# PlakarLabs/plakar

Measured on AMD Instinct MI355X. Metric: GiB/s chunked (device-resident, cut-points out) at 1/2/4/8 MI355X, higher is better.
Workload: dtype u8; 1 GPU; C1: 1x 1 GiB uniform random buffer per GPU (BASELINE configs[1]); bytes_per_gpu=1073741824, global_bytes=1073741824, buffers_per_gpu=1, chunk_params=FASTCDC min 65536 / normal 1048576 / max 4194304, gear=placeholder (v0.0.8 table unavailable; see DESIGN.md), parallelism=independent buffers, 1 rank per GPU x 1, no collective, streams=2

## Files before the change

plakar_amd/csrc/cdc_kernels.hip:

```cpp
#include <hip/hip_ext.h>
#include <hip/hip_runtime.h>

#include <algorithm>
#include <mutex>
#include <type_traits>
#include <vector>

#include "cdc_hostmem.h"
#include "cdc_internal.h"

namespace cdc {

#ifndef CDC_SPIN_SLEEP
#define CDC_SPIN_SLEEP 1
#endif
constexpr int kSpinSleep = CDC_SPIN_SLEEP;

static constexpr uint64_t kNoHit = ~0ull;
static constexpr uint32_t kRawLaneBytes = 512;
static constexpr uint32_t kWarm = 64;

template <int NT, int COPIES = 32>
__device__ __forceinline__ void fill_gear_lds(uint64_t *tab, const uint64_t *gear, uint32_t sh = 0)
{
    static_assert(NT % 64 == 0, "block size");
    constexpr uint32_t kSlots = 256u * COPIES;
    constexpr int kPer = int((kSlots + NT - 1) / NT);
    uint64_t v[kPer];
#pragma unroll
    for (int i = 0; i < kPer; ++i) {
        const uint32_t x = threadIdx.x + uint32_t(i) * NT;
        v[i] = x < kSlots ? gear[x / COPIES] : 0;
    }
#pragma unroll
    for (int i = 0; i < kPer; ++i) {
        const uint32_t x = threadIdx.x + uint32_t(i) * NT;
        if (x < kSlots) tab[x] = v[i] << sh;
    }
}
constexpr uint32_t kWCopies = 8;
constexpr uint32_t kWEntShift = kWCopies == 32 ? 8 : kWCopies == 16 ? 7 : 6;
static_assert(kWCopies == 8 || kWCopies == 16 || kWCopies == 32, "walker table copies");

__device__ __forceinline__ uint64_t lds_gear(const char *tab, uint32_t addr)
{
    return *reinterpret_cast<const uint64_t *>(tab + addr);
}

typedef __attribute__((address_space(3))) const char lds_char;
typedef __attribute__((address_space(1))) const uint64_t g_u64;
typedef __attribute__((address_space(1))) const uint32_t g_u32;
typedef __attribute__((address_space(1))) const uint8_t g_u8;

__device__ __forceinline__ uint64_t lds_gear(const lds_char *tab, uint32_t addr)
{
    return *reinterpret_cast<__attribute__((address_space(3))) const uint64_t *>(tab + addr);
}

template <typename T>
__device__ __forceinline__ T *as_space(uint64_t addr)
{
    return reinterpret_cast<T *>(uintptr_t(addr));
}

__device__ __forceinline__ const lds_char *as_lds(const char *p)
{
    return as_space<const lds_char>(uint32_t(reinterpret_cast<uintptr_t>(p)));
}

__device__ __forceinline__ uint4 gload16(uint64_t a)
{
    const g_u64 *q = as_space<const g_u64>(a);
    const uint64_t x = q[0], y = q[1];
    return make_uint4(uint32_t(x), uint32_t(x >> 32), uint32_t(y), uint32_t(y >> 32));
}

__device__ __forceinline__ uint32_t gear_addr(uint32_t laneoff, uint32_t word, int k)
{
    return __builtin_amdgcn_perm(laneoff, word, 0x0C0C0004u | (uint32_t(k & 3) << 8));
}

template <uint32_t ESH = kWEntShift>
__device__ __forceinline__ uint32_t wgear_addr(uint32_t wlaneoff, uint32_t word, int k)
{
    if constexpr (ESH == 8) return gear_addr(wlaneoff, word, k);
    return (__builtin_amdgcn_ubfe(word, uint32_t(k & 3) * 8u, 8u) << ESH) | wlaneoff;
}

__device__ __forceinline__ uint32_t key_of(uint64_t fp, uint32_t mlo, uint32_t mhi)
{
    return __builtin_amdgcn_bitop3_b32(uint32_t(fp >> 32), mhi, uint32_t(fp) & mlo, 0xEA);
}

__device__ __forceinline__ uint32_t word_of(const uint4 &d, int i)
{
    return i == 0 ? d.x : i == 1 ? d.y : i == 2 ? d.z : d.w;
}

__device__ __forceinline__ uint32_t umin3(uint32_t a, uint32_t b, uint32_t c)
{
    uint32_t r;
    asm("v_min3_u32 %0, %1, %2, %3" : "=v"(r) : "v"(a), "v"(b), "v"(c));
    return r;
}

template <uint32_t ESH = kWEntShift, typename TP>
__device__ __forceinline__ uint32_t roll16_test(const uint4 &d, uint64_t &fp, TP tab,
                                                uint32_t laneoff, uint32_t mlo, uint32_t mhi)
{
    uint32_t acc = 0xFFFFFFFFu;
#pragma unroll
    for (int k = 0; k < 16; ++k) {
        fp = (fp << 1) + lds_gear(tab, wgear_addr<ESH>(laneoff, word_of(d, k >> 2), k));
        acc = min(acc, key_of(fp, mlo, mhi));
    }
    return acc;
}

template <uint32_t ESH = kWEntShift, typename TP>
__device__ __forceinline__ void roll16(const uint4 &d, uint64_t &fp, TP tab,
                                       uint32_t laneoff)
{
#pragma unroll
    for (int k = 0; k < 16; ++k)
        fp = (fp << 1) + lds_gear(tab, wgear_addr<ESH>(laneoff, word_of(d, k >> 2), k));
}

template <uint32_t ESH = kWEntShift, typename TP>
__device__ __forceinline__ uint64_t group_first_hit(const uint4 &d, uint64_t &fp, uint64_t a,
                                                    uint64_t ts, uint64_t te, uint64_t fz,
                                                    TP tab, uint32_t laneoff,
                                                    uint32_t mlo, uint32_t mhi)
// ... 121 lines not shown
    const uint64_t base = (uint64_t(uint32_t(__builtin_amdgcn_readfirstlane(uint32_t(base_in >> 32)))) << 32) |
                          uint32_t(__builtin_amdgcn_readfirstlane(uint32_t(base_in)));
    const uint32_t dst = __builtin_amdgcn_readfirstlane(dst_in);
    uint32_t keep;
    asm volatile("s_nop 4\n\ts_mov_b32 %[keep], m0\n\ts_mov_b32 m0, %[dst]\n\ts_nop 0\n\t"
                 DMA_PIECE_IMM(1, 0) DMA_PIECE_IMM(2, 1024) DMA_PIECE_IMM(3, 2048) DMA_PIECE_IMM(4, 3072)
                 "s_mov_b32 m0, %[keep]\n\ts_nop 1"
                 : [keep] "=&s"(keep)
                 : "v"(offi[0]), "v"(offi[1]), "v"(offi[2]), "v"(offi[3]), [base] "s"(base), [dst] "s"(dst)
                 : "memory");
}

__device__ __forceinline__ uint32_t wave_ticket(uint32_t *p)
{
    const uint32_t old = __hip_atomic_fetch_add(p, (threadIdx.x & 63u) == 0u ? 1u : 0u, __ATOMIC_RELAXED,
                                                __HIP_MEMORY_SCOPE_AGENT);
    return __builtin_amdgcn_readfirstlane(old);
}

__device__ __forceinline__ uint32_t scan_wave_max(uint32_t v)
{
#pragma unroll
    for (int o = 32; o; o >>= 1) v = max(v, uint32_t(__shfl_xor(int(v), o)));
    return __builtin_amdgcn_readfirstlane(v);
}

__device__ __forceinline__ uint32_t rec_cnt(uint64_t rec) { return uint32_t(rec & ((1u << kRecCntBits) - 1)); }
__device__ __forceinline__ uint32_t rec_ent(uint64_t rec, uint32_t e)
{
    return uint32_t(rec >> (kRecCntBits + kRecEntBits * e)) & ((1u << kRecEntBits) - 1);
}

__device__ __forceinline__ void record_hit(uint64_t &rec, int32_t r)
{
    const uint32_t c = rec_cnt(rec);
    if (c < kRunCap) rec |= uint64_t(uint32_t(r)) << (kRecCntBits + kRecEntBits * c);
    if (c < (1u << kRecCntBits) - 1) ++rec;
}

constexpr uint64_t kMaskLSpill = 16;

__device__ bool maskl_needed(const Batch &B, const DevParams &P, const Workspace &W, const BufDesc &D, uint64_t t,
                             uint32_t lane)
{
    const uint64_t sl = B.scan_lane, tb = 64ull * sl;
    const uint64_t start = t * tb, end = min(D.len, start + tb);
    const uint64_t ra = start / sl, rb = (end - 1) / sl;
    const uint64_t gap = P.normal_size - P.min_size - (P.win - 1);
    const uint32_t kc = uint32_t(gap / sl > 2 ? gap / sl - 1 : 1);
    const uint64_t r_lo = ra > kc + kMaskLSpill ? ra - kc - kMaskLSpill : 0;
    const uint64_t *runs = W.runs + 64ull * D.task_base;
    uint32_t cur = 0;
    for (uint64_t r4 = r_lo; r4 <= rb; r4 += 256) {
        uint64_t rec[4];
#pragma unroll
        for (int j = 0; j < 4; ++j) {
            const uint64_t q = r4 + 64u * j + lane;
            rec[j] = q <= rb ? runs[q] : 1ull;
        }
#pragma unroll
        for (int j = 0; j < 4; ++j) {
            const uint64_t r0 = r4 + 64u * j;
            if (r0 > rb) break;
            const uint64_t E = __ballot(rec_cnt(rec[j]) == 0);
            const uint32_t n = uint32_t(min(rb + 1 - r0, uint64_t(64)));
            const uint64_t Z = ~E & (n == 64 ? ~0ull : (1ull << n) - 1);
            const uint64_t below = Z & ((1ull << lane) - 1);
            const uint32_t prev = below ? lane - 1u - (63u - uint32_t(__builtin_clzll(below))) : cur + lane;
            const uint64_t r = r0 + lane;
            bool need = false;
            if (lane < n) {
                if ((E >> lane) & 1ull)
                    need = r >= ra && prev + 1 >= kc;
                else
                    need = prev >= kc && r + kMaskLSpill >= ra;
            }
            if (__ballot(need)) return true;
            cur = Z ? n - 1u - (63u - uint32_t(__builtin_clzll(Z))) : cur + n;
        }
    }
    return false;
}

template <bool kMaskL, bool kFused>
__device__ __forceinline__ void scan_task(const Batch &B, const DevParams &P, const Workspace &W, char *s_lds,
                                          const char *tab, uint32_t task, uint32_t lane, uint32_t wave,
                                          uint32_t laneoff);

template <bool kMaskL, bool kFused = false>
__device__ __forceinline__ void scan_body(const Batch &B, const DevParams &P, const Workspace &W)
{
    static_assert(!(kMaskL && kFused), "k_scan_f builds both indexes, from the MaskS records' side");
    __shared__ __attribute__((aligned(16)))
    char s_lds[kGearLdsBytes + kS2Waves * (kStageBytes + kQBytes) + (kFused ? kFlushTabBytes : 0u)];
    const uint32_t lane = threadIdx.x & 63u;
    const uint32_t wave = __builtin_amdgcn_readfirstlane(threadIdx.x >> 6);
    const uint32_t laneoff = (lane & 31u) << 3;
    const uint32_t task = blockIdx.x * kS2Waves + wave;
    bool act = true;
    if constexpr (kMaskL) {
        act = false;
        if (task < B.total_tasks) {
            uint32_t bb = 0;
            while (bb + 1 < B.nbufs && task >= B.b[bb + 1].task_base) ++bb;
            const BufDesc &Db = B.b[bb];
            const uint64_t t = task - Db.task_base;
            if (t * 64ull * B.scan_lane < Db.len) act = maskl_needed(B, P, W, Db, t, lane);
            if (lane == 0) W.validL[task] = act ? 1u : 0u;
        }
        if (!__syncthreads_or(act ? 1 : 0)) return;
        if (threadIdx.x == 0 && B.maskl_hint)
            __hip_atomic_store(B.maskl_hint, 1u, __ATOMIC_RELAXED, __HIP_MEMORY_SCOPE_SYSTEM);
    }
    if constexpr (!kMaskL) {
        const uint32_t gt = blockIdx.x * blockDim.x + threadIdx.x, nth = gridDim.x * blockDim.x;
        for (uint32_t i = gt; i < B.total_segs; i += nth) {
            W.xg[i] = 0ull;
            W.sg[i] = 0ull;
        }
        if (gt < kMaxBufsPerLaunch + 4)
            W.flags[gt] = gt == kLimitWord ? uint32_t(B.spin_ticks ? B.spin_ticks : kSpinLimit) : 0u;
        if (gt < 2) W.tick[gt] = 0u;
        if (gt < B.nbufs) B.b[gt].res->status = kRowPending;
        if (threadIdx.x == 0) dbg_ts(B, kTsScan + 4 * blockIdx.x);
    }
    uint32_t clk = 0;
    if (!kMaskL && (B.debug & kDbgClk) && blockIdx.x == 0 && threadIdx.x == 0) {
        clk = kTsClk + 4u * uint32_t(atomicAdd(reinterpret_cast<unsigned long long *>(&g_ts[kTsClkN]), 1ull) % kClkRecs);
        g_ts[clk] = __builtin_amdgcn_s_memrealtime();
        g_ts[clk + 1] = __builtin_amdgcn_s_memtime();
    }
    fill_gear_lds<kS2Waves * 64>(reinterpret_cast<uint64_t *>(s_lds), W.gear,
                                 kFused ? P.fm_sh : kMaskL ? P.fl_sh : P.fs_sh);
    if constexpr (kFused) {
        static_assert(kS2Waves * 64 >= 256, "one entry per thread");
        if (threadIdx.x < 256)
            reinterpret_cast<uint64_t *>(s_lds + kGearLdsBytes + kS2Waves * (kStageBytes + kQBytes))[threadIdx.x] =
                W.gear[threadIdx.x] << P.fs_sh;
    }
    __syncthreads();
    if (!kMaskL && threadIdx.x == 0) {
        dbg_ts(B, kTsScan + 4 * blockIdx.x + 1);
        if (blockIdx.x < 4096)
            dbg_ts(B, kTsHw + blockIdx.x,
                   uint64_t(__builtin_amdgcn_s_getreg(20 | (0 << 6) | (15 << 11))) << 32 |
                       uint32_t(__builtin_amdgcn_s_getreg(4 | (0 << 6) | (31 << 11))));
    }
    const char *tab = s_lds;
    if (!act) return;
    const bool persist = !kMaskL && B.persist != 0;
    auto next_task = [&]() { return wave_ticket(W.tick + 2); };
    for (uint32_t cur = persist ? next_task() : task;;) {
        if (cur >= B.total_tasks) break;
        scan_task<kMaskL, kFused>(B, P, W, s_lds, tab, cur, lane, wave, laneoff);
        if (!persist) break;
        cur = next_task();
    }
    if (clk && threadIdx.x == 0) {
        g_ts[clk + 2] = __builtin_amdgcn_s_memrealtime();
        g_ts[clk + 3] = __builtin_amdgcn_s_memtime();
    }
}

template <bool kMaskL, bool kFused>
__device__ __forceinline__ void scan_task(const Batch &B, const DevParams &P, const Workspace &W, char *s_lds,
                                          const char *tab, uint32_t task, uint32_t lane, uint32_t wave,
                                          uint32_t laneoff)
{
    uint32_t b = 0;
    while (b + 1 < B.nbufs && task >= B.b[b + 1].task_base) ++b;
    const BufDesc &D = B.b[b];

    const uint64_t sl = B.scan_lane;
    const uint64_t ub = reinterpret_cast<uint64_t>(D.data);
    const uint64_t lo_ok = ub & ~15ull, hi_ok = (ub + D.len + 15) & ~15ull;
    const uint64_t seg0 = uint64_t(task - D.task_base) * 64u;
    if (seg0 * sl >= D.len) return;
    const int64_t s = int64_t((seg0 + lane) * sl);
    constexpr uint32_t kLead = 128u;
    const uint32_t T = uint32_t((sl + kLead + (ub & 15u) + kStage - 1u) / kStage);
    const uint64_t wb = ((ub + seg0 * sl) & ~15ull) - kLead;
    const uint64_t base = wb > lo_ok ? wb : lo_ok;
    const uint64_t limw = hi_ok - 16u - base;
    const uint32_t lim = limw > 0x7FFFFFFFull ? 0x7FFFFFFFu : uint32_t(limw);
    const uint32_t ring = uint32_t(reinterpret_cast<uintptr_t>(s_lds)) + kGearLdsBytes + wave * kStageBytes;
    static_assert(kStage == 64 && kL == 4, "pair staging: 64-B stages, one slot");
    const uint32_t half = lane >> 5;
    const uint32_t row = lane & 31u, swz = (row >> 1) & 7u;
    uint32_t offi[4];
    uint32_t om = 0;
#pragma unroll
    for (uint32_t j = 0; j < 4; ++j) {
        const uint32_t r = 8u * j + lane / 8u;
        const uint32_t k = (lane % 8u) ^ ((r >> 1) & 7u);
        const uint32_t o = uint32_t((((ub + (seg0 + r) * sl) & ~15ull) - kLead + 16u * k) - base);
        om = max(om, o);
        offi[j] = o - 1024u * j;
    }
    const uint64_t om0 = scan_wave_max(om);
    const uint64_t half_step = 32ull * sl;
    auto issue = [&](auto PC, uint32_t u, auto FC) {
        constexpr uint32_t Q = decltype(PC)::value;
        constexpr bool kFast = decltype(FC)::value;
        const uint64_t adv = uint64_t(kStage) * (u - Q) + (Q ? half_step : 0ull);
#ifdef CDC_DIAG_NO_DMA
        return;
#endif
        if (kFast || om0 + adv <= uint64_t(lim)) {
#ifdef CDC_DIAG_L2
            dma_stage_imm(lo_ok + ((base + adv - lo_ok) & 0x7FFF0ull), ring, offi);
#else
            dma_stage_imm(base + adv, ring, offi);
#endif
        } else {
            uint32_t eff[4];
#pragma unroll
            for (uint32_t j = 0; j < 4; ++j) eff[j] = min(offi[j] + 1024u * j + uint32_t(adv), lim);
            dma_stage(base, ring, eff);
        }
    };
    const char *rowp = s_lds + kGearLdsBytes + wave * kStageBytes + row * 128u;
    auto load_row = [&](uint4 (&first)[4], uint4 (&second)[4]) {
#ifdef CDC_DIAG_NO_ROW
        asm volatile("" : "+v"(first[0].x), "+v"(second[0].x));
        return;
#endif
#pragma unroll
        for (uint32_t g = 0; g < 4; ++g) first[g] = *reinterpret_cast<const uint4 *>(rowp + 16u * (g ^ swz));
#pragma unroll
        for (uint32_t g = 0; g < 4; ++g) second[g] = *reinterpret_cast<const uint4 *>(rowp + 16u * ((g + 4) ^ swz));
    };
    const uint32_t TT = T + 1;
    const int32_t lag = int32_t(kStage * half);
    const uint32_t vhi = to_vgpr(kFused ? P.fm_mi : kMaskL ? P.fl_hi : P.fs_hi);
    const uint32_t xlo = kMaskL ? P.fl_lo : P.fs_lo, xhi = kMaskL ? P.fl_hi : P.fs_hi;
    const int64_t rel0 = int64_t(((ub + uint64_t(s)) & ~15ull) - kLead) - int64_t(ub);
    using C0 = std::integral_constant<uint32_t, 0>;
    using C1 = std::integral_constant<uint32_t, 1>;
    using Gen = std::integral_constant<bool, false>;
    using Steady = std::integral_constant<bool, true>;

    uint4 A[4] = {}, Bv[4] = {};
#ifdef CDC_DIAG_WAITS
    uint64_t wsum = 0;
    uint32_t nrc = 0;
    const uint64_t tk0 = __builtin_amdgcn_s_memtime();
    const uint64_t rt0 = __builtin_amdgcn_s_memrealtime();
#endif
    static_assert(kLead >= 2 * kStage, "stage 0 must be pure warm-up for both halves");
    issue(C0{}, 0, Gen{});
    wait_vmcnt<0>();
    if (half == 0) load_row(A, Bv);
    asm volatile("s_waitcnt lgkmcnt(0)" ::: "memory");
    if (1 < TT) issue(C1{}, 1, Gen{});
    if (1 < TT) {
        wait_vmcnt<0>();
        if (half == 1) load_row(Bv, A);
        asm volatile("s_waitcnt lgkmcnt(0)" ::: "memory");
        if (2 < TT) issue(C0{}, 2, Gen{});
    }
    uint64_t gv[2][16];
#pragma unroll
    for (int k = 0; k < 16; ++k) gv[0][k] = lds_gear(tab, gear_addr(laneoff, word_of(Bv[0], k >> 2), k));
    uint64_t fp = 0;
    uint64_t rec = 0;
    uint64_t recL = 0;
    const int32_t rr0 = int32_t(rel0 - s) - lag;
    uint64_t *const qf = reinterpret_cast<uint64_t *>(s_lds + kGearLdsBytes + kS2Waves * kStageBytes + wave * kQBytes);
    uint32_t *const qm = reinterpret_cast<uint32_t *>(qf + kQCap);
    static_assert(kQCap == 64, "one flush pass: item j in lane j");
    uint32_t qn = 0;
    const char *const ftab = s_lds + kGearLdsBytes + kS2Waves * (kStageBytes + kQBytes);
    auto rgear = [&](const uint4 &d, int k) -> uint64_t {
        if constexpr (kFused)
            return lds_gear(ftab, __builtin_amdgcn_ubfe(word_of(d, k >> 2), uint32_t(k & 3) * 8u, 8u) << 3);
        else
            return lds_gear(tab, gear_addr(laneoff, word_of(d, k >> 2), k));
    };
    auto flush = [&]() {
        {
            const bool v = lane < qn;
            const uint32_t meta = qm[v ? lane : 0u];
            const uint32_t owner = meta >> 24;
            const int32_t r0 = int32_t(meta & 0xFFFFFFu) - 256;
            const int64_t so = int64_t((seg0 + owner) * sl);
            const int32_t ln = so < int64_t(D.len) ? int32_t(min(int64_t(sl), int64_t(D.len) - so)) : 0;
            const uint64_t a = ub + uint64_t(so + r0);
            auto clamp16 = [&](uint64_t x) { return min(max(x, lo_ok), hi_ok - 16u); };
            const uint4 d0 = gload16(clamp16(a)), d1 = gload16(clamp16(a + 16u));
            uint64_t f = 0;
            if constexpr (kFused) {
                uint4 dw[4];
#pragma unroll
                for (int h = 0; h < 4; ++h) dw[h] = gload16(clamp16(a - 64u + 16u * uint32_t(h)));
#pragma unroll
                for (int k = 0; k < 64; ++k) f = (f << 1) + rgear(dw[k >> 4], k & 15);
            } else {
                f = qf[v ? lane : 0u];
            }
            uint32_t miss = 0, missL = 0;
#pragma unroll
            for (int k = 0; k < 32; ++k) {
                f = (f << 1) + rgear(k < 16 ? d0 : d1, k & 15);
                miss |= min(key_of(f, xlo, xhi), 1u) << k;
                if constexpr (kFused) missL |= min(key_of(f, P.fm_llo, P.fm_lhi), 1u) << k;
            }
            const int32_t lo = r0 < 0 ? -r0 : 0, hi = ln - r0;
            uint32_t vm = lo >= 32 ? 0u : (0xFFFFFFFFu << lo);
            vm &= hi >= 32 ? 0xFFFFFFFFu : (hi <= 0 ? 0u : (1u << hi) - 1u);
            const uint32_t hm = v ? ~miss & vm : 0u;
            const uint32_t hmL = kFused && v ? ~missL & vm : 0u;
            uint64_t todo = __ballot(hm != 0 || hmL != 0);
            while (todo) {
                const int i = int(__builtin_ctzll(todo));
                todo &= todo - 1;
                const uint32_t o = uint32_t(__builtin_amdgcn_readlane(int(owner), i));
                const int32_t ri = __builtin_amdgcn_readlane(r0, i);
                uint32_t m = uint32_t(__builtin_amdgcn_readlane(int(hm), i));
                uint32_t mL = kFused ? uint32_t(__builtin_amdgcn_readlane(int(hmL), i)) : 0u;
                if (lane == o) {
                    for (; m; m &= m - 1) record_hit(rec, ri + int32_t(__builtin_ctz(m)));
                    if constexpr (kFused)
                        for (; mL; mL &= mL - 1) record_hit(recL, ri + int32_t(__builtin_ctz(mL)));
                }
            }
        }
        qn = 0;
    };
    uint64_t f0 = 0;
    uint32_t acc = 0xFFFFFFFFu;
    auto stage = [&](auto PC, auto SC, uint32_t t, uint4 (&cur_d)[4], uint4 (&nxt_d)[4]) {
        constexpr uint32_t Q = decltype(PC)::value;
        constexpr bool kSteady = decltype(SC)::value;
#pragma unroll
        for (uint32_t gi = 0; gi < kGroups; ++gi) {
            if (gi + 1 == kGroups && (kSteady || t + 1 < TT)) {
#ifdef CDC_DIAG_WAITS
                const uint64_t w0 = __builtin_amdgcn_s_memtime();
                wait_vmcnt<0>();
                wsum += __builtin_amdgcn_s_memtime() - w0;
#else
                wait_vmcnt<0>();
#endif
                if (half != Q) load_row(nxt_d, cur_d);
                asm volatile("" ::: "memory");
            }
            const uint4 nx = gi + 1 < kGroups ? cur_d[gi + 1] : nxt_d[0];
            uint64_t (&cg)[16] = gv[gi & 1];
            uint64_t (&ng)[16] = gv[(gi + 1) & 1];
            if ((gi & 1) == 0) {
                f0 = fp;
                acc = 0xFFFFFFFFu;
            }
#pragma unroll
            for (int q = 0; q < 4; ++q) {
#pragma unroll
                for (int k = 4 * q; k < 4 * q + 4; k += 2) {
                    const uint32_t a0 = gear_addr(laneoff, word_of(nx, k >> 2), k);
                    fp = (fp << 1) + cg[k];
                    ng[k] = lds_gear(tab, a0);
                    const uint32_t k0 = uint32_t(fp >> 32) & vhi;
                    const uint32_t a1 = gear_addr(laneoff, word_of(nx, (k + 1) >> 2), k + 1);
                    fp = (fp << 1) + cg[k + 1];
                    ng[k + 1] = lds_gear(tab, a1);
                    acc = umin3(acc, k0, uint32_t(fp >> 32) & vhi);
                    __builtin_amdgcn_sched_barrier(0);
                }
                __builtin_amdgcn_sched_barrier(0);
                if (q == 1 && gi + 1 == kGroups && (kSteady || t + 2 < TT)) {
                    asm volatile("s_waitcnt lgkmcnt(8)" ::: "memory");
                    issue(PC, t + 2, SC);
                    __builtin_amdgcn_sched_barrier(0);
                }
            }
            if (gi & 1) {
#ifndef CDC_DIAG_NO_RECHECK
                const uint64_t fm = __ballot(acc == 0);
#ifdef CDC_DIAG_WAITS
                nrc += fm ? 1u : 0u;
#endif
                if (fm) [[unlikely]] {
                    const uint32_t nq = uint32_t(__popcll(fm));
                    if (qn + nq > kQCap) flush();
                    if (acc == 0) {
                        const uint32_t idx =
                            qn + __builtin_amdgcn_mbcnt_hi(uint32_t(fm >> 32), __builtin_amdgcn_mbcnt_lo(uint32_t(fm), 0u));
                        const int32_t r0 = rr0 + int32_t(kStage * t + 16u * (gi - 1));
                        if constexpr (!kFused) qf[idx] = f0;
                        qm[idx] = uint32_t(r0 + 256) | (lane << 24);
                    }
                    qn += nq;
                }
#else
                rec += acc == 0 ? 1u : 0u;
#endif
            }
        }
    };
    if (1 < TT) stage(C1{}, Gen{}, 1, Bv, A);
    const int64_t room = int64_t(lim) - int64_t(om0) - int64_t(half_step);
    const int64_t tf = room >= 128 ? room / 64 - 1 : 0;
    const uint32_t t_steady = uint32_t(max<int64_t>(2, min<int64_t>(int64_t(TT) - 3, tf)));
    uint32_t t = 2;
    for (; t < t_steady; t += 2) {
        stage(C0{}, Steady{}, t, A, Bv);
        stage(C1{}, Steady{}, t + 1, Bv, A);
    }
    for (; t < TT; t += 2) {
        stage(C0{}, Gen{}, t, A, Bv);
        if (t + 1 < TT) stage(C1{}, Gen{}, t + 1, Bv, A);
    }
    if (qn) flush();
    if (s < int64_t(D.len)) (kMaskL ? W.runsL : W.runs)[64ull * D.task_base + seg0 + lane] = rec;
    if constexpr (kFused) {
        if (s < int64_t(D.len)) W.runsL[64ull * D.task_base + seg0 + lane] = recL;
        if (lane == 0) W.validL[task] = 1u;
    }
    if (!kMaskL && lane == 0) dbg_ts(B, kTsScan + 4 * blockIdx.x + 2 + (wave & 1));
#ifdef CDC_DIAG_WAITS
    if (lane == 0 && 8 * task + 7 < 8 * 16384) {
        uint64_t *o = g_ts + kTsRes + 8 * task;
        o[0] = wsum;
        o[1] = __builtin_amdgcn_s_memtime() - tk0;
        o[2] = rt0;
        o[3] = __builtin_amdgcn_s_memrealtime();
        o[4] = __builtin_amdgcn_s_getreg(4 | (0 << 6) | (31 << 11));
        o[5] = __builtin_amdgcn_s_getreg(20 | (0 << 6) | (15 << 11));
        o[6] = nrc;
        o[7] = wave;
    }
#endif
}

#ifndef CDC_SCAN_LB
#define CDC_SCAN_LB (kS2Waves * 64)
#endif
__global__ __launch_bounds__(CDC_SCAN_LB) void k_scan(const Batch B, const DevParams P, const Workspace W)
{
    scan_body<false>(B, P, W);
}

__global__ __launch_bounds__(kS2Waves * 64) void k_scan_l(const Batch B, const DevParams P, const Workspace W)
{
    scan_body<true>(B, P, W);
}

__global__ __launch_bounds__(CDC_SCAN_LB) void k_scan_f(const Batch B, const DevParams P, const Workspace W)
{
    scan_body<false, true>(B, P, W);
}

constexpr uint32_t kProbeWaves = 4;

__global__ __launch_bounds__(kProbeWaves * 64) void k_maskl_probe(const Batch B, const DevParams P, const Workspace W)
{
    const uint32_t lane = threadIdx.x & 63u;
    const uint32_t task = blockIdx.x * kProbeWaves + __builtin_amdgcn_readfirstlane(threadIdx.x >> 6);
    if (task >= B.total_tasks) return;
    uint32_t b = 0;
    while (b + 1 < B.nbufs && task >= B.b[b + 1].task_base) ++b;
    const BufDesc &D = B.b[b];
    const uint64_t t = task - D.task_base;
    if (t * 64ull * B.scan_lane >= D.len) return;
    if (maskl_needed(B, P, W, D, t, lane) && lane == 0 && B.maskl_hint)
        __hip_atomic_store(B.maskl_hint, 1u, __ATOMIC_RELAXED, __HIP_MEMORY_SCOPE_SYSTEM);
}

constexpr int kDppRowShr = 0x110;

template <int N>
__device__ __forceinline__ uint64_t dpp_shr64_zero(uint64_t v)
{
    const uint32_t lo = __builtin_amdgcn_update_dpp(0u, uint32_t(v), kDppRowShr + N, 0xF, 0xF, true);
    const uint32_t hi = __builtin_amdgcn_update_dpp(0u, uint32_t(v >> 32), kDppRowShr + N, 0xF, 0xF, true);
    return (uint64_t(hi) << 32) | lo;
}

template <int N>
__device__ __forceinline__ uint32_t dpp_shr32_keep(uint32_t v)
{
    return __builtin_amdgcn_update_dpp(v, v, kDppRowShr + N, 0xF, 0xF, false);
}

__device__ __forceinline__ uint64_t readlane64(uint64_t v, int l)
{
    const uint32_t lo = uint32_t(__builtin_amdgcn_readlane(uint32_t(v), l));
    const uint32_t hi = uint32_t(__builtin_amdgcn_readlane(uint32_t(v >> 32), l));
    return (uint64_t(hi) << 32) | lo;
}

__device__ __forceinline__ uint32_t wave_min_u32(uint32_t x)
{
    x = min(x, dpp_shr32_keep<1>(x));
    x = min(x, dpp_shr32_keep<2>(x));
    x = min(x, dpp_shr32_keep<4>(x));
    x = min(x, dpp_shr32_keep<8>(x));
    const uint32_t r0 = uint32_t(__builtin_amdgcn_readlane(x, 15));
    const uint32_t r1 = uint32_t(__builtin_amdgcn_readlane(x, 31));
    const uint32_t r2 = uint32_t(__builtin_amdgcn_readlane(x, 47));
    const uint32_t r3 = uint32_t(__builtin_amdgcn_readlane(x, 63));
    return min(min(r0, r1), min(r2, r3));
}

__global__ __launch_bounds__(64) void k_selftest_wave(const uint64_t *in, uint32_t *out)
{
    __shared__ uint64_t s_in[64];
    __shared__ uint64_t s_v[64];
    const uint32_t j = threadIdx.x;
    uint64_t g = in[j];
    s_in[j] = g;
    uint64_t v = g;
    v += dpp_shr64_zero<1>(v) << 1;
    v += dpp_shr64_zero<2>(v) << 2;
    v += dpp_shr64_zero<4>(v) << 4;
    v += dpp_shr64_zero<8>(v) << 8;
    s_v[j] = v;
    {
        const uint64_t f15 = readlane64(v, 15);
        const uint64_t f31 = readlane64(v, 31) + (f15 << 16);
        const uint64_t f47 = readlane64(v, 47) + (f31 << 16);
        const uint32_t row = j >> 4;
        const uint64_t carry = row == 0 ? 0ull : row == 1 ? f15 : row == 2 ? f31 : f47;
// ... 944 lines not shown
    }
    if (l0) dbg_ts(B, kTsRes + 8 * g + 3);
    const bool on = E == q && !aborted;
    const bool fb = B.force_fallback != 0;
    if (on && !fb && nodes > 0) {
        auto node_at = [&](uint32_t u) -> uint64_t {
            const uint64_t fj = shfl64(jv, min(u, 63u));
            const uint64_t fc = shfl64(cv, min(u >= c2 ? k + (u - c2) : 0u, 63u));
            return u >= nodes ? ex : (u < c2 ? fj : fc);
        };
        for (uint32_t t0 = 0; t0 < nodes; t0 += 64) {
            const uint32_t t = t0 + lane;
            const uint64_t v = node_at(t), s = node_at(t + 1);
            if (t < nodes) {
                if (s == kUndet) {
                    st_rlx(&D.res->consumed, v);
                } else {
                    if (O + t < D.cap) put_cut(D.out + O + t, v, s - v);
                    if (s >= C.len) st_rlx(&D.res->consumed, C.len);
                }
            }
        }
        drain_stores();
    }
    const uint32_t Eq = on ? (conv == kConvEnd ? kSegEnd : conv + 1) : E;
    const uint64_t Oq = O + (on ? cuts : 0ull);
    if (aborted) {
        if (l0) st_rlx(W.sg + g, kKindAbort);
        abort_rows(B, lane);
        return;
    }
    if (l0) {
        st_rlx(W.sg + g, kKindIncl | (uint64_t(Eq) << 38) | Oq);
        dbg_ts(B, kTsRes + 8 * g + 4);
        if (!(B.debug & kDbgGraph)) {
            dbg_ts(B, kTsRes + 8 * g + 5, G.n);
            dbg_ts(B, kTsRes + 8 * g + 6, exact);
            dbg_ts(B, kTsRes + 8 * g + 7, c2);
        }
    }
    if (q + 1 != D.nseg) return;
    if (fb || __hip_atomic_load(W.flags + b, __ATOMIC_RELAXED, __HIP_MEMORY_SCOPE_AGENT)) {
        for (uint32_t p0 = 0; p0 < q; p0 += 64) {
            const uint32_t p = p0 + lane;
            SpinGuard sp;
            while (__ballot(p < q && (ld_rlx(sgb + min(p, q - 1)) >> 62) < 2)) {
                if (!sp.ok(W.flags, kWaitLast, g, p0)) {
                    aborted = true;
                    break;
                }
                __builtin_amdgcn_s_sleep(kSpinSleep);
            }
            if (aborted || __ballot(p < q && (ld_rlx(sgb + min(p, q - 1)) >> 62) == 3)) {
                abort_rows(B, lane);
                return;
            }
        }
        if (__hip_atomic_load(W.flags + b, __ATOMIC_RELAXED, __HIP_MEMORY_SCOPE_AGENT) || fb) {
            resolve_sequential(C, P, D);
            return;
        }
    }
    if (l0) {
        const bool ab = __hip_atomic_load(W.flags + kAbortWord, __ATOMIC_RELAXED, __HIP_MEMORY_SCOPE_AGENT) != 0;
        st_rlx(&D.res->ncuts, Oq <= D.cap ? Oq : D.cap);
        st_rlx(&D.res->needed, Oq);
        settle_row(D.res, ab ? CDC_E_DEVICE : Oq <= D.cap ? CDC_OK : CDC_E_NOSPACE);
    }
}

__device__ __forceinline__ void write_empty_rows(const Batch &B, uint32_t lane)
{
    for (uint32_t i = lane; i < B.nbufs; i += 64) {
        if (B.b[i].nseg == 0) {
            B.b[i].res->ncuts = 0;
            B.b[i].res->consumed = 0;
            B.b[i].res->needed = 0;
            if (B.total_tasks) settle_row(B.b[i].res, CDC_OK);
            else B.b[i].res->status = CDC_OK;
        }
    }
}

#ifdef CDC_RESOLVE_WAVES_PER_EU
#define CDC_RESOLVE_ATTR __attribute__((amdgpu_waves_per_eu(CDC_RESOLVE_WAVES_PER_EU)))
#else
#define CDC_RESOLVE_ATTR
#endif
__global__ CDC_RESOLVE_ATTR __launch_bounds__(kWalkWavesPerWG * 64) void k_resolve(const Batch B, const DevParams P, const Workspace W)
{
    __builtin_amdgcn_s_setprio(3);
    __shared__ uint64_t s_tab[256 * kWCopies];
    __shared__ uint64_t s_grec[kWalkWavesPerWG][kGRecs];
    __shared__ uint64_t s_gx[kWalkWavesPerWG][kGExtra];
    __shared__ uint32_t s_ticket;
    const uint32_t wave = threadIdx.x >> 6, lane = threadIdx.x & 63u;
    if (threadIdx.x == 0) s_ticket = __hip_atomic_fetch_add(W.tick, 1u, __ATOMIC_RELAXED, __HIP_MEMORY_SCOPE_AGENT);
    fill_gear_lds<kWalkWavesPerWG * 64, kWCopies>(s_tab, W.gear);
    __syncthreads();
    if (blockIdx.x == 0 && wave == 0) write_empty_rows(B, lane);
    const uint32_t g = uint32_t(__builtin_amdgcn_readfirstlane(s_ticket)) * kWalkWavesPerWG + wave;
    if (g < B.total_segs)
        resolve_segment(B, P, W, g, reinterpret_cast<const char *>(s_tab), graph_lds(s_grec[wave], s_gx[wave]));
}

constexpr uint32_t kStreamThreads = 256;

__global__ __launch_bounds__(kStreamThreads) void k_stream_read(const uint4 *p, uint64_t n16, uint32_t *sink)
{
    const uint64_t stride = uint64_t(gridDim.x) * kStreamThreads;
    uint64_t i = uint64_t(blockIdx.x) * kStreamThreads + threadIdx.x;
    uint32_t x = 0;
    for (; i + 3 * stride < n16; i += 4 * stride) {
        const uint4 a = p[i], b = p[i + stride], c = p[i + 2 * stride], d = p[i + 3 * stride];
        x ^= a.x ^ a.y ^ a.z ^ a.w ^ b.x ^ b.y ^ b.z ^ b.w ^ c.x ^ c.y ^ c.z ^ c.w ^ d.x ^ d.y ^ d.z ^ d.w;
    }
    for (; i < n16; i += stride) {
        const uint4 a = p[i];
        x ^= a.x ^ a.y ^ a.z ^ a.w;
    }
    for (int o = 32; o; o >>= 1) x ^= uint32_t(__shfl_xor(int(x), o));
    if ((threadIdx.x & 63u) == 0) atomicXor(sink + blockIdx.x, x);
}

__global__ __launch_bounds__(kStreamThreads) void k_stream_read_nt(const uint4 *p, uint64_t n16, uint32_t *sink)
{
    const uint64_t waves = uint64_t(gridDim.x) * (kStreamThreads / 64);
    const uint64_t w = uint64_t(blockIdx.x) * (kStreamThreads / 64) + (threadIdx.x >> 6);
    const uint32_t lane = threadIdx.x & 63u;
    uint32_t x = 0;
    const uint64_t pieces = n16 / 512;
    for (uint64_t q = w; q < pieces; q += waves) {
        typedef uint32_t u32x4 __attribute__((ext_vector_type(4)));
        const u32x4 *b = reinterpret_cast<const u32x4 *>(p + q * 512 + lane);
        u32x4 v[8];
#pragma unroll
        for (int k = 0; k < 8; ++k) v[k] = __builtin_nontemporal_load(b + 64 * k);
#pragma unroll
        for (int k = 0; k < 8; ++k) x ^= v[k].x ^ v[k].y ^ v[k].z ^ v[k].w;
    }
    for (uint64_t i = pieces * 512 + uint64_t(blockIdx.x) * kStreamThreads + threadIdx.x; i < n16;
         i += uint64_t(gridDim.x) * kStreamThreads) {
        const uint4 a = p[i];
        x ^= a.x ^ a.y ^ a.z ^ a.w;
    }
    for (int o = 32; o; o >>= 1) x ^= uint32_t(__shfl_xor(int(x), o));
    if (lane == 0) atomicXor(sink + blockIdx.x, x);
}

constexpr uint32_t kStreamLdsWaves = 4;

__global__ __launch_bounds__(kStreamLdsWaves * 64) void k_stream_read_lds(const uint8_t *p, uint64_t len, uint32_t *sink)
{
    __shared__ __attribute__((aligned(16))) char lds[kStreamLdsWaves * 2 * 4096];
    const uint32_t lane = threadIdx.x & 63u, wave = __builtin_amdgcn_readfirstlane(threadIdx.x >> 6);
    const uint64_t nw = uint64_t(gridDim.x) * kStreamLdsWaves, w = uint64_t(blockIdx.x) * kStreamLdsWaves + wave;
    const uint64_t steps = len / 4096, per = (steps + nw - 1) / nw;
    const uint64_t s0 = w * per, s1 = min(steps, s0 + per);
    uint32_t off[4];
#pragma unroll
    for (uint32_t j = 0; j < 4; ++j) off[j] = 1024u * j + 16u * lane;
    const uint32_t slot = uint32_t(reinterpret_cast<uintptr_t>(lds)) + wave * 8192u;
    for (uint64_t q = s0; q < s1; ++q) {
        dma_stage(reinterpret_cast<uint64_t>(p) + q * 4096, slot + uint32_t((q - s0) & 1) * 4096u, off);
        asm volatile("s_waitcnt vmcnt(4)" ::: "memory");
    }
    asm volatile("s_waitcnt vmcnt(0)" ::: "memory");
    __syncthreads();
    if (threadIdx.x == 0) sink[blockIdx.x] = *reinterpret_cast<const uint32_t *>(lds);
}

int launch_stream_read(const void *d_buf, uint64_t len, int reps, double *best_us, double *median_us, void *stream)
{
    if (!best_us || !median_us) return CDC_E_INVALID;
    hipStream_t st = reinterpret_cast<hipStream_t>(stream);
    const uint64_t n16 = len / 16;
    if (n16 == 0 || reps <= 0 || (reinterpret_cast<uintptr_t>(d_buf) & 15u)) return CDC_E_INVALID;
    int cus = 0, dev = 0;
    if (hipGetDevice(&dev) != hipSuccess ||
// ... 265 lines not shown
```

Before: 5127 GiB/s.

## Halve scan gear prefetch depth and cap k_scan VGPRs for higher occupancy

Templates the scan loop on how many gear gathers stay in flight and defaults k_scan to 8 instead of 16. The ring buffer is rotated so the row reload and the next stage issue move earlier in each group. k_scan is capped at 56 VGPRs via amdgpu_num_vgpr with launch bounds of 1024, and the flush path reloads data in 16-byte pieces inside a tight loop to save registers. The aim is more resident waves to hide LDS and global latency, at the cost of less per-wave memory-level parallelism and a risk of register spills.

```diff
diff --git a/plakar_amd/csrc/cdc_kernels.hip b/plakar_amd/csrc/cdc_kernels.hip
--- a/plakar_amd/csrc/cdc_kernels.hip
+++ b/plakar_amd/csrc/cdc_kernels.hip
@@ -48,6 +48,8 @@
 }
 
 typedef __attribute__((address_space(3))) const char lds_char;
+typedef uint32_t u32x4 __attribute__((ext_vector_type(4)));
+typedef __attribute__((address_space(3))) const u32x4 lds_u32x4;
 typedef __attribute__((address_space(1))) const uint64_t g_u64;
 typedef __attribute__((address_space(1))) const uint32_t g_u32;
 typedef __attribute__((address_space(1))) const uint8_t g_u8;
@@ -335,16 +337,16 @@
     return false;
 }
 
-template <bool kMaskL, bool kFused>
+template <bool kMaskL, bool kFused, int kDepth>
 __device__ __forceinline__ void scan_task(const Batch &B, const DevParams &P, const Workspace &W, char *s_lds,
                                           const char *tab, uint32_t task, uint32_t lane, uint32_t wave,
                                           uint32_t laneoff);
 
-template <bool kMaskL, bool kFused = false>
+template <bool kMaskL, bool kFused = false, int kDepth = 16>
 __device__ __forceinline__ void scan_body(const Batch &B, const DevParams &P, const Workspace &W)
 {
     static_assert(!(kMaskL && kFused), "k_scan_f builds both indexes, from the MaskS records' side");
-    __shared__ __attribute__((aligned(16)))
+    __shared__ __attribute__((aligned(kDepth < 16 ? 128 : 16)))
     char s_lds[kGearLdsBytes + kS2Waves * (kStageBytes + kQBytes) + (kFused ? kFlushTabBytes : 0u)];
     const uint32_t lane = threadIdx.x & 63u;
     const uint32_t wave = __builtin_amdgcn_readfirstlane(threadIdx.x >> 6);
@@ -405,7 +407,7 @@
     auto next_task = [&]() { return wave_ticket(W.tick + 2); };
     for (uint32_t cur = persist ? next_task() : task;;) {
         if (cur >= B.total_tasks) break;
-        scan_task<kMaskL, kFused>(B, P, W, s_lds, tab, cur, lane, wave, laneoff);
+        scan_task<kMaskL, kFused, kDepth>(B, P, W, s_lds, tab, cur, lane, wave, laneoff);
         if (!persist) break;
         cur = next_task();
     }
@@ -415,13 +417,19 @@
     }
 }
 
-template <bool kMaskL, bool kFused>
+template <bool kMaskL, bool kFused, int kDepth>
 __device__ __forceinline__ void scan_task(const Batch &B, const DevParams &P, const Workspace &W, char *s_lds,
                                           const char *tab, uint32_t task, uint32_t lane, uint32_t wave,
                                           uint32_t laneoff)
 {
+    static_assert(kDepth == 8 || kDepth == 16, "gathers in flight: half a 16-byte group or a whole one");
+    if constexpr (kDepth < 16) {
+        asm volatile("" : "+v"(lane));
+        laneoff = (lane & 31u) << 3;
+    }
     uint32_t b = 0;
     while (b + 1 < B.nbufs && task >= B.b[b + 1].task_base) ++b;
+    if constexpr (kDepth < 16) b = __builtin_amdgcn_readfirstlane(b);
     const BufDesc &D = B.b[b];
 
     const uint64_t sl = B.scan_lane;
@@ -450,7 +458,15 @@
         om = max(om, o);
         offi[j] = o - 1024u * j;
     }
-    const uint64_t om0 = scan_wave_max(om);
+    uint64_t om0;
+    if constexpr (kDepth < 16) {
+#pragma unroll
+        for (uint32_t o = 32; o; o >>= 1)
+            om = max(om, uint32_t(__builtin_amdgcn_ds_bpermute(int((lane ^ o) << 2), int(om))));
+        om0 = uint32_t(__builtin_amdgcn_readfirstlane(om));
+    } else {
+        om0 = scan_wave_max(om);
+    }
     const uint64_t half_step = 32ull * sl;
     auto issue = [&](auto PC, uint32_t u, auto FC) {
         constexpr uint32_t Q = decltype(PC)::value;
@@ -473,11 +489,22 @@
         }
     };
     const char *rowp = s_lds + kGearLdsBytes + wave * kStageBytes + row * 128u;
+    const uint32_t row0 = ring + row * 128u + 16u * swz;
     auto load_row = [&](uint4 (&first)[4], uint4 (&second)[4]) {
 #ifdef CDC_DIAG_NO_ROW
         asm volatile("" : "+v"(first[0].x), "+v"(second[0].x));
         return;
 #endif
+        if constexpr (kDepth < 16) {
+            uint32_t p0 = row0;
+            asm volatile("" : "+v"(p0));
+#pragma unroll
+            for (uint32_t g = 0; g < 8; ++g) {
+                const u32x4 x = *as_space<lds_u32x4>(p0 ^ (16u * g));
+                (g < 4 ? first[g] : second[g - 4]) = make_uint4(x.x, x.y, x.z, x.w);
+            }
+            return;
+        }
 #pragma unroll
         for (uint32_t g = 0; g < 4; ++g) first[g] = *reinterpret_cast<const uint4 *>(rowp + 16u * (g ^ swz));
 #pragma unroll
@@ -512,9 +539,9 @@
         asm volatile("s_waitcnt lgkmcnt(0)" ::: "memory");
         if (2 < TT) issue(C0{}, 2, Gen{});
     }
-    uint64_t gv[2][16];
-#pragma unroll
-    for (int k = 0; k < 16; ++k) gv[0][k] = lds_gear(tab, gear_addr(laneoff, word_of(Bv[0], k >> 2), k));
+    uint64_t gv[kDepth];
+#pragma unroll
+    for (int k = 0; k < kDepth; ++k) gv[k] = lds_gear(tab, gear_addr(laneoff, word_of(Bv[0], k >> 2), k));
     uint64_t fp = 0;
     uint64_t rec = 0;
     uint64_t recL = 0;
@@ -530,7 +557,8 @@
         else
             return lds_gear(tab, gear_addr(laneoff, word_of(d, k >> 2), k));
     };
-    auto flush = [&]() {
+    auto flush = [&](auto TC) {
+        constexpr bool kTight = decltype(TC)::value;
         {
             const bool v = lane < qn;
             const uint32_t meta = qm[v ? lane : 0u];
@@ -540,7 +568,11 @@
             const int32_t ln = so < int64_t(D.len) ? int32_t(min(int64_t(sl), int64_t(D.len) - so)) : 0;
             const uint64_t a = ub + uint64_t(so + r0);
             auto clamp16 = [&](uint64_t x) { return min(max(x, lo_ok), hi_ok - 16u); };
-            const uint4 d0 = gload16(clamp16(a)), d1 = gload16(clamp16(a + 16u));
+            uint4 d0 = {}, d1 = {};
+            if constexpr (!kTight) {
+                d0 = gload16(clamp16(a));
+                d1 = gload16(clamp16(a + 16u));
+            }
             uint64_t f = 0;
             if constexpr (kFused) {
                 uint4 dw[4];
@@ -552,11 +584,32 @@
                 f = qf[v ? lane : 0u];
             }
             uint32_t miss = 0, missL = 0;
-#pragma unroll
-            for (int k = 0; k < 32; ++k) {
-                f = (f << 1) + rgear(k < 16 ? d0 : d1, k & 15);
-                miss |= min(key_of(f, xlo, xhi), 1u) << k;
-                if constexpr (kFused) missL |= min(key_of(f, P.fm_llo, P.fm_lhi), 1u) << k;
+            if constexpr (!kTight) {
+#pragma unroll
+                for (int k = 0; k < 32; ++k) {
+                    f = (f << 1) + rgear(k < 16 ? d0 : d1, k & 15);
+                    miss |= min(key_of(f, xlo, xhi), 1u) << k;
+                    if constexpr (kFused) missL |= min(key_of(f, P.fm_llo, P.fm_lhi), 1u) << k;
+                }
+            } else {
+#pragma unroll
+                for (int k0 = 0; k0 < 32; k0 += 4) {
+                    if (k0 == 0 || k0 == 16) d0 = gload16(clamp16(a + uint32_t(k0)));
+                    uint64_t g[4];
+                    __builtin_amdgcn_sched_barrier(0);
+#pragma unroll
+                    for (int k = 0; k < 4; ++k) g[k] = rgear(d0, (k0 + k) & 15);
+                    __builtin_amdgcn_sched_barrier(0);
+                    uint32_t m4 = 0, m4L = 0;
+#pragma unroll
+                    for (int k = 0; k < 4; ++k) {
+                        f = (f << 1) + g[k];
+                        m4 |= min(key_of(f, xlo, xhi), 1u) << k;
+                        if constexpr (kFused) m4L |= min(key_of(f, P.fm_llo, P.fm_lhi), 1u) << k;
+                    }
+                    miss |= m4 << k0;
+                    if constexpr (kFused) missL |= m4L << k0;
+                }
             }
             const int32_t lo = r0 < 0 ? -r0 : 0, hi = ln - r0;
             uint32_t vm = lo >= 32 ? 0u : (0xFFFFFFFFu << lo);
@@ -587,40 +640,43 @@
         constexpr bool kSteady = decltype(SC)::value;
 #pragma unroll
         for (uint32_t gi = 0; gi < kGroups; ++gi) {
-            if (gi + 1 == kGroups && (kSteady || t + 1 < TT)) {
-#ifdef CDC_DIAG_WAITS
-                const uint64_t w0 = __builtin_amdgcn_s_memtime();
-                wait_vmcnt<0>();
-                wsum += __builtin_amdgcn_s_memtime() - w0;
-#else
-                wait_vmcnt<0>();
-#endif
-                if (half != Q) load_row(nxt_d, cur_d);
-                asm volatile("" ::: "memory");
-            }
-            const uint4 nx = gi + 1 < kGroups ? cur_d[gi + 1] : nxt_d[0];
-            uint64_t (&cg)[16] = gv[gi & 1];
-            uint64_t (&ng)[16] = gv[(gi + 1) & 1];
+            const bool last = gi + 1 == kGroups;
+            constexpr int kTurn = 16 - kDepth;
             if ((gi & 1) == 0) {
                 f0 = fp;
                 acc = 0xFFFFFFFFu;
             }
 #pragma unroll
             for (int q = 0; q < 4; ++q) {
+                if (4 * q == kTurn && last && (kSteady || t + 1 < TT)) {
+#ifdef CDC_DIAG_WAITS
+                    const uint64_t w0 = __builtin_amdgcn_s_memtime();
+                    wait_vmcnt<0>();
+                    wsum += __builtin_amdgcn_s_memtime() - w0;
+#else
+                    wait_vmcnt<0>();
+#endif
+                    if (half != Q) load_row(nxt_d, cur_d);
+                    asm volatile("" ::: "memory");
+                }
 #pragma unroll
                 for (int k = 4 * q; k < 4 * q + 4; k += 2) {
-                    const uint32_t a0 = gear_addr(laneoff, word_of(nx, k >> 2), k);
-                    fp = (fp << 1) + cg[k];
-                    ng[k] = lds_gear(tab, a0);
+                    const int j = k + kDepth;
+                    const uint4 &src = j < 16 ? cur_d[gi] : last ? nxt_d[0] : cur_d[gi + 1];
+                    const uint32_t w = word_of(src, (j & 15) >> 2);
+                    uint64_t &g0 = gv[k % kDepth], &g1 = gv[(k + 1) % kDepth];
+                    const uint32_t a0 = gear_addr(laneoff, w, j);
+                    fp = (fp << 1) + g0;
+                    g0 = lds_gear(tab, a0);
                     const uint32_t k0 = uint32_t(fp >> 32) & vhi;
-                    const uint32_t a1 = gear_addr(laneoff, word_of(nx, (k + 1) >> 2), k + 1);
-                    fp = (fp << 1) + cg[k + 1];
-                    ng[k + 1] = lds_gear(tab, a1);
+                    const uint32_t a1 = gear_addr(laneoff, w, j + 1);
+                    fp = (fp << 1) + g1;
+                    g1 = lds_gear(tab, a1);
                     acc = umin3(acc, k0, uint32_t(fp >> 32) & vhi);
                     __builtin_amdgcn_sched_barrier(0);
                 }
                 __builtin_amdgcn_sched_barrier(0);
-                if (q == 1 && gi + 1 == kGroups && (kSteady || t + 2 < TT)) {
+                if (4 * q + 4 == kTurn + 8 && last && (kSteady || t + 2 < TT)) {
                     asm volatile("s_waitcnt lgkmcnt(8)" ::: "memory");
                     issue(PC, t + 2, SC);
                     __builtin_amdgcn_sched_barrier(0);
@@ -634,7 +690,7 @@
 #endif
                 if (fm) [[unlikely]] {
                     const uint32_t nq = uint32_t(__popcll(fm));
-                    if (qn + nq > kQCap) flush();
+                    if (qn + nq > kQCap) flush(std::integral_constant<bool, (kDepth < 16)>{});
                     if (acc == 0) {
                         const uint32_t idx =
                             qn + __builtin_amdgcn_mbcnt_hi(uint32_t(fm >> 32), __builtin_amdgcn_mbcnt_lo(uint32_t(fm), 0u));
@@ -663,7 +719,7 @@
         stage(C0{}, Gen{}, t, A, Bv);
         if (t + 1 < TT) stage(C1{}, Gen{}, t + 1, Bv, A);
     }
-    if (qn) flush();
+    if (qn) flush(std::false_type{});
     if (s < int64_t(D.len)) (kMaskL ? W.runsL : W.runs)[64ull * D.task_base + seg0 + lane] = rec;
     if constexpr (kFused) {
         if (s < int64_t(D.len)) W.runsL[64ull * D.task_base + seg0 + lane] = recL;
@@ -688,9 +744,16 @@
 #ifndef CDC_SCAN_LB
 #define CDC_SCAN_LB (kS2Waves * 64)
 #endif
-__global__ __launch_bounds__(CDC_SCAN_LB) void k_scan(const Batch B, const DevParams P, const Workspace W)
-{
-    scan_body<false>(B, P, W);
+#ifndef CDC_SCAN_VGPRS
+#define CDC_SCAN_VGPRS 112
+#endif
+#ifndef CDC_SCAN_DEPTH
+#define CDC_SCAN_DEPTH 8
+#endif
+static_assert(CDC_SCAN_VGPRS % 8 == 0 && CDC_SCAN_VGPRS >= 104 && CDC_SCAN_VGPRS <= 128, "k_scan's register budget");
+__global__ __attribute__((amdgpu_num_vgpr(CDC_SCAN_VGPRS / 2))) __launch_bounds__(1024) void k_scan(const Batch B, const DevParams P, const Workspace W)
+{
+    scan_body<false, false, CDC_SCAN_DEPTH>(B, P, W);
 }
 
 __global__ __launch_bounds__(kS2Waves * 64) void k_scan_l(const Batch B, const DevParams P, const Workspace W)
@@ -1801,19 +1864,17 @@
     }
 }
 
-#ifdef CDC_RESOLVE_WAVES_PER_EU
-#define CDC_RESOLVE_ATTR __attribute__((amdgpu_waves_per_eu(CDC_RESOLVE_WAVES_PER_EU)))
-#else
-#define CDC_RESOLVE_ATTR
+#ifndef CDC_RESOLVE_PRIO
+#define CDC_RESOLVE_PRIO 3
 #endif
-__global__ CDC_RESOLVE_ATTR __launch_bounds__(kWalkWavesPerWG * 64) void k_resolve(const Batch B, const DevParams P, const Workspace W)
-{
-    __builtin_amdgcn_s_setprio(3);
+__global__ __launch_bounds__(kWalkWavesPerWG * 64) void k_resolve(const Batch B, const DevParams P, const Workspace W)
+{
+    __builtin_amdgcn_s_setprio(CDC_RESOLVE_PRIO);
     __shared__ uint64_t s_tab[256 * kWCopies];
     __shared__ uint64_t s_grec[kWalkWavesPerWG][kGRecs];
     __shared__ uint64_t s_gx[kWalkWavesPerWG][kGExtra];
     __shared__ uint32_t s_ticket;
-    const uint32_t wave = threadIdx.x >> 6, lane = threadIdx.x & 63u;
+    const uint32_t wave = __builtin_amdgcn_readfirstlane(threadIdx.x >> 6), lane = threadIdx.x & 63u;
     if (threadIdx.x == 0) s_ticket = __hip_atomic_fetch_add(W.tick, 1u, __ATOMIC_RELAXED, __HIP_MEMORY_SCOPE_AGENT);
     fill_gear_lds<kWalkWavesPerWG * 64, kWCopies>(s_tab, W.gear);
     __syncthreads();
```

New measurement: 5230 GiB/s, median of 6. 2.0% higher.
